# facebookresearch/hyperreel

Hardware: NVIDIA H100
Metric: Mrays/s at 65k-ray x 32-sample batch (higher is better)
Workload: dtype f32 (sample net bf16x3 split on wgmma, fp32 accumulate)

## Files before the change

hyperreel_b200/csrc/hr_mlp.cuh:

```cuda
#pragma once
#include <cuda_runtime.h>
#include "hyperreel_b200.h"

namespace hr {

struct MlpSimtPack {
  const float* Wt[HR_MAX_LAYERS];
  const float* bias[HR_MAX_LAYERS];
  int Kp[HR_MAX_LAYERS];
  int Np[HR_MAX_LAYERS];
  int in_pad;
  int n_layers;
  int skip;
};

#define HR_TC_MAX_PASSES 40
struct TcPass {
  int layer;
  int n;
  int first_chunk;
  int n_chunks;
  int bias_off;
  int is_final;
  int out_col0;
  int wait_a;
};
struct MlpTcPack {
  const void* wpack;
  const float* bias;
  long long wpack_bytes;
  int n_passes;
  int bias_count;
  int in_chunks;
  TcPass passes[HR_TC_MAX_PASSES];
};

size_t mlp_simt_smem_bytes(const MlpSimtPack& pk, int W);
cudaError_t launch_mlp_simt(const hr_config& cfg, const MlpSimtPack& pk, const float* rays, float* heads,
                            long long n, int num_sms, cudaStream_t stream);

cudaError_t launch_mlp_tc2(const hr_config& cfg, const MlpTcPack& pk, const float* rays, float* heads, long long n,
                           int num_sms, cudaStream_t stream, float* rays_copy = nullptr);

struct TrainSave {
  float* enc;
  float* act;
  long long act_stride;
  int ld_enc;
};
cudaError_t launch_mlp_tc2_train(const hr_config& cfg, const MlpTcPack& pk, const float* rays, float* heads, long long n,
                                 int num_sms, cudaStream_t stream, const TrainSave& sv);

struct TrainNetLayout {
  size_t enc, act, act_stride, dlast, dy[2], part, dbpart, total;
  int ld_enc;
};
TrainNetLayout train_net_layout(const hr_config& c, long long n, int num_sms);
cudaError_t train_net_backward(const hr_config& c, const MlpSimtPack& simt, long long n, float* const* weight,
                               float* const* bias, uint8_t* ws, int num_sms, cudaStream_t st);
}

struct hr_handle;
struct hr_params;
namespace hr {
int pack_mlp_tc2(hr_handle* h, const hr_config& c, MlpTcPack& pk, size_t& alloc_bytes, int& alloc_bias,
                 const float* const* w_dev, const float* const* b_dev, cudaStream_t st);
void free_mlp_tc2(hr_handle* h);
}
```

hyperreel_b200/csrc/hr_mlp_tc2.cu:

```cuda
#include <cuda.h>
#include <cuda_bf16.h>

#include <cstdio>
#include <cstdlib>
#include <cstring>

#include "hr_encode.cuh"
#include "hr_handle.h"
#include "hr_tc_prims.cuh"

namespace hr {

namespace tc2 {
using namespace tc;

constexpr int NSTAGE = 4;
constexpr int STAGE_BYTES = 8192;
constexpr int KSTEP_BYTES = 4096;
constexpr int CONSUMERS = 2;
constexpr int NTHREADS = (CONSUMERS + 1) * 128;
constexpr int PRODUCER_REGS = 40;
constexpr int CONSUMER_REGS = 232;
static_assert(128 * PRODUCER_REGS + CONSUMERS * 128 * CONSUMER_REGS <= 65536, "register file");

constexpr int A_BYTES = 16 * KSTEP_BYTES;
constexpr int OFF_AHI = 0;
constexpr int OFF_ALO = OFF_AHI + A_BYTES;
constexpr int X_BYTES = 4 * KSTEP_BYTES;
constexpr int OFF_X = OFF_ALO + A_BYTES;
constexpr int OFF_B = OFF_X + 2 * X_BYTES;
constexpr int OFF_BAR = OFF_B + CONSUMERS * NSTAGE * STAGE_BYTES;
constexpr int SMEM_BYTES = OFF_BAR + 128;
static_assert(SMEM_BYTES <= 232448, "shared memory budget");

constexpr int BAR_FULL = 0;
constexpr int BAR_EMPTY = BAR_FULL + CONSUMERS * NSTAGE;
static_assert((BAR_EMPTY + CONSUMERS * NSTAGE) * 8 <= 128, "barrier block");

constexpr int NB_RET = 3;
constexpr int NB_WR = 5;
constexpr int NB_XW = 7;
constexpr int NB_XR = 9;

}

template <int W, bool SAVE>
__global__ void __launch_bounds__(tc2::NTHREADS, 1)
mlp_tc2_kernel(const __grid_constant__ hr_config cfg, const __grid_constant__ MlpTcPack pk, const float* __restrict__ rays,
               float* __restrict__ heads, long long n_rays, float* __restrict__ rays_copy, const TrainSave sv) {
  using namespace tc2;
  constexpr int WH = W / 2;
  constexpr int NACC = WH / 2;
  constexpr int NK = W / 16;
  constexpr int NKH = NK / 2;
  constexpr int IMG_BYTES = WH * 64;
  constexpr int KPS = STAGE_BYTES / IMG_BYTES;
  static_assert(KPS * IMG_BYTES == STAGE_BYTES && NKH % KPS == 0 && NK * KSTEP_BYTES <= A_BYTES, "pass width");
  extern __shared__ __align__(128) uint8_t smem[];
  const uint32_t sbase = smem_u32(smem);
  const int tid = threadIdx.x, warp = tid >> 5, lane = tid & 31;
  auto bar = [&](int slot) -> uint32_t { return sbase + OFF_BAR + slot * 8; };

  {
    const char* w = reinterpret_cast<const char*>(pk.wpack);
    const long long lines = pk.wpack_bytes >> 7;
    for (long long i = (long long)blockIdx.x * NTHREADS + tid; i < lines; i += (long long)gridDim.x * NTHREADS)
      asm volatile("prefetch.global.L2 [%0];" ::"l"(w + i * 128));
  }
  for (int i = tid; i < (2 * X_BYTES) / 16; i += NTHREADS)
    reinterpret_cast<uint4*>(smem + OFF_X)[i] = make_uint4(0u, 0u, 0u, 0u);
  if (tid == 0) {
    for (int s = 0; s < CONSUMERS * NSTAGE; ++s) { mbar_init(bar(BAR_FULL + s), 1); mbar_init(bar(BAR_EMPTY + s), 1); }
    asm volatile("fence.mbarrier_init.release.cluster;" ::: "memory");
  }
  __syncthreads();

  const long long n_tiles = (n_rays + BM - 1) / BM;
  const int n_passes = pk.n_passes;
  const long long n_iters = ((long long)blockIdx.x < n_tiles) ? (n_tiles - 1 - blockIdx.x) / gridDim.x + 1 : 0;

  if (warp >= CONSUMERS * 4) {
    setmaxnreg_dec<PRODUCER_REGS>();
    const int g = warp - CONSUMERS * 4;
    if (g < CONSUMERS && lane == 0) {
      const long long half_bytes = pk.wpack_bytes / CONSUMERS;
      const int n_stages = (int)(half_bytes / STAGE_BYTES);
      const uint32_t full0 = bar(BAR_FULL + g * NSTAGE), empty0 = bar(BAR_EMPTY + g * NSTAGE);
      const uint32_t ring = sbase + OFF_B + (uint32_t)(g * NSTAGE * STAGE_BYTES);
      uint32_t stage = 0, phase = 0;
      for (long long iter = 0; iter < n_iters; ++iter) {
        const uint8_t* src = reinterpret_cast<const uint8_t*>(pk.wpack) + g * half_bytes;
        for (int i = 0; i < n_stages; ++i) {
          mbar_wait(empty0 + stage * 8, phase ^ 1);
          mbar_expect_tx(full0 + stage * 8, STAGE_BYTES);
          bulk_g2s(ring + stage * STAGE_BYTES, src, STAGE_BYTES, full0 + stage * 8);
          src += STAGE_BYTES;
          if (++stage == NSTAGE) { stage = 0; phase ^= 1; }
        }
      }
    }
    return;
  }

  setmaxnreg_inc<CONSUMER_REGS>();
  const int wg = warp >> 2;
  const int wt = tid & 127;
  const int rowq = (warp & 3) * 16 + (lane >> 2);
  const int q2 = (lane & 3) * 2;
  const int col0 = wg * WH;
  const int in_chunks = pk.in_chunks;
  const int L = cfg.mlp_layers;
  const uint32_t x_lo_off = (uint32_t)(2 * in_chunks * KSTEP_BYTES);
  const uint32_t full0 = bar(BAR_FULL + wg * NSTAGE), empty0 = bar(BAR_EMPTY + wg * NSTAGE);
  const uint32_t ring = sbase + OFF_B + (uint32_t)(wg * NSTAGE * STAGE_BYTES);
  const bool vec_ok = ((reinterpret_cast<uintptr_t>(rays) | reinterpret_cast<uintptr_t>(rays_copy)) & 15) == 0;
  int x_last = 0;
  for (int p = 0; p < n_passes; ++p)
    if (pk.passes[p].first_chunk == 0) x_last = p;
  uint32_t stage = 0, phase = 0;
  int pend = -1;

  float acc[2][NACC];

  auto stage_begin = [&]() {
    mbar_wait(full0 + stage * 8, phase);
    wgmma_fence();
    acc_fence(acc[0]);
    acc_fence(acc[1]);
  };
  auto stage_end = [&]() {
    wgmma_commit();
    acc_fence(acc[0]);
    acc_fence(acc[1]);
    wgmma_wait<1>();
    if (pend >= 0 && wt == 0) mbar_arrive(empty0 + pend * 8);
    pend = (int)stage;
    if (++stage == NSTAGE) { stage = 0; phase ^= 1; }
  };
  auto b_img = [&](int sub) -> uint32_t { return ring + stage * STAGE_BYTES + (uint32_t)sub * IMG_BYTES; };
  auto kstep = [&](uint32_t a, uint32_t a_lo, uint32_t b, uint32_t scale) {
    const uint64_t bh = gmma_desc(b, WH * 16, 128), bl = gmma_desc(b + WH * 32, WH * 16, 128);
    const uint64_t ah0 = gmma_desc(a, 2048, 128), ah1 = gmma_desc(a + 1024, 2048, 128);
    const uint64_t al0 = gmma_desc(a + a_lo, 2048, 128), al1 = gmma_desc(a + a_lo + 1024, 2048, 128);
    wgmma_ss(acc[0], ah0, bh, scale);
    wgmma_ss(acc[1], ah1, bh, scale);
    wgmma_ss(acc[0], al0, bh, 1u);
    wgmma_ss(acc[1], al1, bh, 1u);
    wgmma_ss(acc[0], ah0, bl, 1u);
    wgmma_ss(acc[1], ah1, bl, 1u);
  };
  auto run_pass = [&](const TcPass& P, bool fresh, bool x_ret, bool ret) {
    int ki = 0;
    if (P.first_chunk == 0) {
      for (; ki < 2 * in_chunks; ki += KPS) {
        stage_begin();
#pragma unroll
        for (int sub = 0; sub < KPS; ++sub)
          kstep(sbase + OFF_X + (uint32_t)(ki + sub) * KSTEP_BYTES, x_lo_off, b_img(sub), (ki + sub) != 0 ? 1u : 0u);
        stage_end();
      }
    }
    if (P.first_chunk + P.n_chunks > in_chunks) {
      const uint32_t scale0 = ki != 0 ? 1u : 0u;
#pragma unroll
      for (int kk = 0; kk < NK; ++kk) {
        if (kk % KPS == 0) {
          if (fresh && kk == (wg == 0 ? NKH : 0)) {
            if (wg == 0) pair_arrive(NB_WR + 0);
            pair_wait(NB_WR + (wg ^ 1));
          }
          stage_begin();
        }
        kstep(sbase + OFF_AHI + (uint32_t)kk * KSTEP_BYTES, OFF_ALO - OFF_AHI, b_img(kk % KPS), kk != 0 ? 1u : scale0);
        if (kk % KPS == KPS - 1) {
          stage_end();
          if (x_ret && kk == KPS - 1) pair_arrive(NB_XR + wg);
          if (ret && wg == 1 && kk == NKH + KPS - 1) pair_arrive(NB_RET + 1);
        }
      }
    }
  };
  auto drain = [&]() {
    wgmma_wait<0>();
    acc_fence(acc[0]);
    acc_fence(acc[1]);
    if (pend >= 0 && wt == 0) mbar_arrive(empty0 + pend * 8);
    pend = -1;
  };
  const int st_row = (warp & 3) * 16 + 8 * ((lane >> 3) & 1) + (lane & 7);
  const uint32_t st_off = ks_slot(st_row, lane >> 4);
  auto store_hidden = [&](const float* bias, int layer, long long tile) {
#pragma unroll
    for (int kk = 0; kk < NKH; ++kk) {
      float2 b[2];
#pragma unroll
      for (int jj = 0; jj < 2; ++jj) b[jj] = __ldg(reinterpret_cast<const float2*>(bias + col0 + 8 * (2 * kk + jj) + q2));
#pragma unroll
      for (int m = 0; m < 2; ++m) {
        uint32_t hi[4], lo[4];
#pragma unroll
        for (int jj = 0; jj < 2; ++jj) {
          const int j = 2 * kk + jj, k = col0 + 8 * j + q2;
#pragma unroll
          for (int h = 0; h < 2; ++h) {
            float t0 = acc[m][4 * j + 2 * h] + b[jj].x, t1 = acc[m][4 * j + 2 * h + 1] + b[jj].y;
            t0 = fmaxf(t0, t0 * cfg.leaky_slope);
            t1 = fmaxf(t1, t1 * cfg.leaky_slope);
            split2(t0, t1, hi[2 * jj + h], lo[2 * jj + h]);
            if constexpr (SAVE) {
              const long long ray = tile * BM + 64 * m + rowq + 8 * h;
              if (ray < n_rays) *reinterpret_cast<float2*>(sv.act + layer * sv.act_stride + ray * W + k) = make_float2(t0, t1);
            }
          }
        }
        const uint32_t a = sbase + st_off + (uint32_t)m * 1024u + (uint32_t)(wg * NKH + kk) * KSTEP_BYTES;
        stmatrix_x4(a + OFF_AHI, hi);
        stmatrix_x4(a + OFF_ALO, lo);
      }
    }
  };
  auto encode = [&](long long tile, bool after_x) {
    if (after_x) pair_wait(NB_XR + (wg ^ 1));
    const int r = wg * 64 + (wt & 63), part = wt >> 6;
    const long long ray = tile * BM + r;
    auto put = [&](int k, float val) {
      if constexpr (SAVE) {
        if (ray < n_rays) sv.enc[ray * sv.ld_enc + k] = val;
      }
      const __nv_bfloat16 hi = __float2bfloat16_rn(val);
      const __nv_bfloat16 lo = __float2bfloat16_rn(val - __bfloat162float(hi));
      const uint32_t off = (uint32_t)(k >> 4) * KSTEP_BYTES + ks_slot(r, (k >> 3) & 1) + (uint32_t)(k & 7) * 2u;
      *reinterpret_cast<__nv_bfloat16*>(smem + OFF_X + off) = hi;
      *reinterpret_cast<__nv_bfloat16*>(smem + OFF_X + x_lo_off + off) = lo;
    };
    if (ray < n_rays) {
      float rbuf[16];
      const float* src = rays + ray * cfg.c_in;
      if (cfg.c_in == 8 && vec_ok) {
        const float4 a = *reinterpret_cast<const float4*>(src), b = *reinterpret_cast<const float4*>(src + 4);
        rbuf[0] = a.x; rbuf[1] = a.y; rbuf[2] = a.z; rbuf[3] = a.w; rbuf[4] = b.x; rbuf[5] = b.y; rbuf[6] = b.z; rbuf[7] = b.w;
        if (rays_copy != nullptr && part == 0) {
          float4* dst = reinterpret_cast<float4*>(rays_copy + ray * 8);
          dst[0] = a; dst[1] = b;
        }
      } else {
        for (int i = 0; i < cfg.c_in; ++i) rbuf[i] = src[i];
        if (rays_copy != nullptr && part == 0)
          for (int i = 0; i < cfg.c_in; ++i) rays_copy[ray * cfg.c_in + i] = rbuf[i];
      }
      encode_ray_features(cfg, rbuf, part, 2, put);
      if constexpr (SAVE) {
        if (part == 0)
          for (int k = cfg.mlp_in; k < sv.ld_enc; ++k) sv.enc[ray * sv.ld_enc + k] = 0.0f;
      }
    } else if (part == 0) {
      for (int k = 0; k < cfg.mlp_in; ++k) put(k, 0.0f);
    }
    fence_async_smem();
    wg_sync(1 + wg);
    pair_arrive(NB_XW + wg);
  };

  for (long long iter = 0; iter < n_iters; ++iter) {
    const long long tile = iter * gridDim.x + blockIdx.x;
    const bool more = iter + 1 < n_iters;
    if (iter == 0) encode(tile, false);
    pair_wait(NB_XW + (wg ^ 1));
    for (int p = 0; p < n_passes; ++p) {
      const TcPass& P = pk.passes[p];
      const bool reads_a = P.first_chunk + P.n_chunks > in_chunks;
      const bool hidden = p < L - 1;
      const bool ret = reads_a && (hidden || (p == n_passes - 1 && more));
      const bool x_ret = p == x_last && more;
      run_pass(P, reads_a && P.wait_a != 0, x_ret, ret);
      drain();
      if (x_ret && !reads_a) pair_arrive(NB_XR + wg);
      if (ret && wg == 0) pair_arrive(NB_RET + 0);
      if (hidden) {
        wg_sync(1 + wg);
        if (p > 0 || iter > 0) pair_wait(NB_RET + (wg ^ 1));
        store_hidden(pk.bias + P.bias_off, p, tile);
        fence_async_smem();
        wg_sync(1 + wg);
        if (wg == 1) pair_arrive(NB_WR + 1);
      } else {
        const float* bias = pk.bias + P.bias_off;
        if constexpr (SAVE) {
#pragma unroll
          for (int m = 0; m < 2; ++m)
#pragma unroll
            for (int h = 0; h < 2; ++h) {
              const long long ray = tile * BM + 64 * m + rowq + 8 * h;
              if (ray >= n_rays) continue;
              float* row = heads + ray * cfg.mlp_out;
#pragma unroll
              for (int j = 0; j < WH / 8; ++j) {
                const int c = col0 + 8 * j + q2;
                if (P.out_col0 + c < cfg.mlp_out) {
                  const float2 b = __ldg(reinterpret_cast<const float2*>(bias + c));
                  const int c0 = P.out_col0 + c, c1 = c0 + 1, S = cfg.n_samples;
                  row[(c0 % S) * cfg.head_stride + c0 / S] = acc[m][4 * j + 2 * h] + b.x;
                  row[(c1 % S) * cfg.head_stride + c1 / S] = acc[m][4 * j + 2 * h + 1] + b.y;
                }
              }
            }
        } else {
          const bool odd = (lane & 1) != 0;
#pragma unroll
          for (int jp = 0; jp < WH / 16; ++jp) {
            const int j = 2 * jp, c = col0 + 8 * j + q2;
            const float2 b0 = __ldg(reinterpret_cast<const float2*>(bias + c));
            const float2 b1 = __ldg(reinterpret_cast<const float2*>(bias + c + 8));
#pragma unroll
            for (int m = 0; m < 2; ++m)
#pragma unroll
              for (int h = 0; h < 2; ++h) {
                const float2 v0 = make_float2(acc[m][4 * j + 2 * h] + b0.x, acc[m][4 * j + 2 * h + 1] + b0.y);
                const float2 v1 = make_float2(acc[m][4 * j + 4 + 2 * h] + b1.x, acc[m][4 * j + 4 + 2 * h + 1] + b1.y);
                const float2 send = odd ? v0 : v1;
                const float2 recv = make_float2(__shfl_xor_sync(0xffffffffu, send.x, 1), __shfl_xor_sync(0xffffffffu, send.y, 1));
                const int c4 = odd ? c + 6 : c;
                const long long ray = tile * BM + 64 * m + rowq + 8 * h;
                if (ray < n_rays && P.out_col0 + c4 < cfg.mlp_out)
                  *reinterpret_cast<float4*>(heads + ray * cfg.mlp_out + P.out_col0 + c4) =
                      odd ? make_float4(recv.x, recv.y, v1.x, v1.y) : make_float4(v0.x, v0.y, recv.x, recv.y);
              }
          }
        }
      }
      if (x_ret) encode(tile + gridDim.x, true);
    }
  }
}

int pack_mlp_tc2(hr_handle* h, const hr_config& c, MlpTcPack& pk, size_t& alloc_bytes, int& alloc_bias,
                 const float* const* w_dev, const float* const* b_dev, cudaStream_t st) {
  const int W = c.mlp_width;
  if (W != 128 && W != 256) return hr_fail("tensor-core sample net: hidden width must be 128 or 256 (got %d)", W);
  if (c.mlp_in > 64) return hr_fail("tensor-core sample net: encoded input wider than 64 features (%d)", c.mlp_in);
  const int in_chunks = (c.mlp_in + 31) / 32;
  const int L = c.mlp_layers;
  MlpTcPack np_{};
  np_.in_chunks = in_chunks;
  int np = 0, bias_off = 0;
  size_t bytes = 0;
  for (int l = 0; l < L; ++l) {
    const bool last = (l == L - 1);
    const int out = last ? c.mlp_out : W;
    const int n_parts = (out + W - 1) / W;
    for (int part = 0; part < n_parts; ++part) {
      if (np >= HR_TC_MAX_PASSES) return hr_fail("tensor-core sample net: too many passes (%d output columns)", c.mlp_out);
      TcPass& P = np_.passes[np++];
      const bool reads_input = (l == 0 || l == c.mlp_skip);
      P.layer = l;
      P.n = W;
      P.first_chunk = reads_input ? 0 : in_chunks;
      P.n_chunks = (l == 0) ? in_chunks : (W / 32 + (reads_input ? in_chunks : 0));
      P.bias_off = bias_off;
      P.is_final = last ? 1 : 0;
      P.out_col0 = part * W;
      P.wait_a = (part == 0) ? 1 : 0;
      bias_off += P.n;
      bytes += (size_t)P.n_chunks * 2 * P.n * 64;
    }
  }
  np_.n_passes = np;
  np_.bias_count = bias_off;
  np_.wpack_bytes = (long long)bytes;
  if (alloc_bytes != bytes || alloc_bias != bias_off || !pk.wpack) {
    if (pk.wpack) cudaFree(const_cast<void*>(pk.wpack));
    if (pk.bias) cudaFree(const_cast<float*>(pk.bias));
    pk.wpack = nullptr; pk.bias = nullptr;
    alloc_bytes = 0; alloc_bias = 0;
    void* wp = nullptr; float* bp = nullptr;
    cudaError_t e = cudaMalloc(&wp, bytes);
    if (e != cudaSuccess) return hr_fail("cudaMalloc(tc weights %zu): %s", bytes, cudaGetErrorString(e));
    e = cudaMalloc((void**)&bp, (size_t)bias_off * sizeof(float));
    if (e != cudaSuccess) { cudaFree(wp); return hr_fail("cudaMalloc(tc bias): %s", cudaGetErrorString(e)); }
    np_.wpack = wp; np_.bias = bp;
    alloc_bytes = bytes; alloc_bias = bias_off;
    e = (W == 256) ? cudaFuncSetAttribute(mlp_tc2_kernel<256, false>, cudaFuncAttributeMaxDynamicSharedMemorySize, tc2::SMEM_BYTES)
                   : cudaFuncSetAttribute(mlp_tc2_kernel<128, false>, cudaFuncAttributeMaxDynamicSharedMemorySize, tc2::SMEM_BYTES);
    if (e != cudaSuccess) return hr_fail("cudaFuncSetAttribute(mlp_tc2_kernel): %s", cudaGetErrorString(e));
  } else {
    np_.wpack = pk.wpack; np_.bias = pk.bias;
  }
  pk = np_;
  uint8_t* wp = (uint8_t*)const_cast<void*>(pk.wpack);
  float* bp = const_cast<float*>(pk.bias);
  const int WH = W / 2;
  for (int half = 0; half < 2; ++half) {
    size_t off = (size_t)half * (bytes / 2);
    for (int p = 0; p < np; ++p) {
      const TcPass& P = pk.passes[p];
      const int l = P.layer;
      const bool last = (l == L - 1), skip = (l == c.mlp_skip), first = (l == 0);
      const int in_src = first ? c.mlp_in : (skip ? c.mlp_in + W : W);
      launch_pack_tc_pass(w_dev[l], b_dev[l], wp + off, bp + P.bias_off + half * WH, WH, P.first_chunk, P.n_chunks, in_src,
                          c.mlp_in, skip ? 1 : 0, in_chunks, last ? c.mlp_out : W, last ? c.n_samples : 0, c.head_stride,
                          P.out_col0 + half * WH, st);
      off += (size_t)P.n_chunks * 2 * WH * 64;
    }
  }
  cudaError_t e = cudaGetLastError();
  if (e != cudaSuccess) return hr_fail("tc pack launch failed: %s", cudaGetErrorString(e));
  return 0;
}

void free_mlp_tc2(hr_handle* h) {
  if (h->tc.wpack) cudaFree(const_cast<void*>(h->tc.wpack));
  if (h->tc.bias) cudaFree(const_cast<float*>(h->tc.bias));
  h->tc.wpack = nullptr; h->tc.bias = nullptr;
  h->tc_alloc_bytes = 0; h->tc_alloc_bias = 0;
  if (h->tc_pre.wpack) cudaFree(const_cast<void*>(h->tc_pre.wpack));
  if (h->tc_pre.bias) cudaFree(const_cast<float*>(h->tc_pre.bias));
  h->tc_pre.wpack = nullptr; h->tc_pre.bias = nullptr;
  h->tc_pre_alloc_bytes = 0; h->tc_pre_alloc_bias = 0;
}

cudaError_t launch_mlp_tc2(const hr_config& cfg, const MlpTcPack& pk, const float* rays, float* heads, long long n, int num_sms,
                           cudaStream_t stream, float* rays_copy) {
  if ((cfg.mlp_out % 4) != 0 || ((uintptr_t)heads % 16) != 0) return cudaErrorInvalidValue;
  long long tiles = (n + tc::BM - 1) / tc::BM;
  int grid = (int)(tiles < num_sms ? tiles : num_sms);
  if (grid < 1) grid = 1;
  if (cfg.mlp_width == 256)
    mlp_tc2_kernel<256, false><<<grid, tc2::NTHREADS, tc2::SMEM_BYTES, stream>>>(cfg, pk, rays, heads, n, rays_copy, TrainSave{});
  else if (cfg.mlp_width == 128)
    mlp_tc2_kernel<128, false><<<grid, tc2::NTHREADS, tc2::SMEM_BYTES, stream>>>(cfg, pk, rays, heads, n, rays_copy, TrainSave{});
  else
    return cudaErrorInvalidValue;
  return cudaGetLastError();
}

cudaError_t launch_mlp_tc2_train(const hr_config& cfg, const MlpTcPack& pk, const float* rays, float* heads, long long n,
                                 int num_sms, cudaStream_t stream, const TrainSave& sv) {
  if ((cfg.mlp_out % 4) != 0) return cudaErrorInvalidValue;
  long long tiles = (n + tc::BM - 1) / tc::BM;
  int grid = (int)(tiles < num_sms ? tiles : num_sms);
  if (grid < 1) grid = 1;
  auto kern = cfg.mlp_width == 256 ? mlp_tc2_kernel<256, true> : mlp_tc2_kernel<128, true>;
  if (cfg.mlp_width != 256 && cfg.mlp_width != 128) return cudaErrorInvalidValue;
  cudaError_t e = cudaFuncSetAttribute(kern, cudaFuncAttributeMaxDynamicSharedMemorySize, tc2::SMEM_BYTES);
  if (e != cudaSuccess) return e;
  kern<<<grid, tc2::NTHREADS, tc2::SMEM_BYTES, stream>>>(cfg, pk, rays, heads, n, nullptr, sv);
  return cudaGetLastError();
}

}
```

hyperreel_b200/csrc/hr_tc_pack.cu:

```cuda
#include <cuda_bf16.h>

#include "hr_tc_prims.cuh"

namespace hr {

__global__ void pack_tc_pass(const float* __restrict__ W, const float* __restrict__ b, uint8_t* __restrict__ dst,
                             float* __restrict__ bias_dst, int n, int first_chunk, int n_chunks, int in_src, int mlp_in,
                             int is_skip, int in_chunks, int out_rows, int perm_S, int perm_stride, int out_col0) {
  const long long total = (long long)n_chunks * 2 * n * 16;
  for (long long i = blockIdx.x * (long long)blockDim.x + threadIdx.x; i < total + n; i += (long long)gridDim.x * blockDim.x) {
    if (i >= total) {
      int nn = (int)(i - total);
      int ncol = out_col0 + nn;
      float v = 0.0f;
      if (ncol < out_rows) {
        int ns = perm_S > 0 ? (ncol % perm_S) * perm_stride + (ncol / perm_S) : ncol;
        v = b[ns];
      }
      bias_dst[nn] = v;
      continue;
    }
    int kk = (int)(i % 16);
    int nn = (int)((i / 16) % n);
    int img = (int)(i / (16LL * n));
    int c = first_chunk + img / 2, ks = img % 2;
    int kc = ks * 16 + kk;
    int ksrc = -1;
    if (c < in_chunks) {
      const int kin = c * 32 + kc;
      if (kin < mlp_in) ksrc = kin;
    } else {
      int hcol = (c - in_chunks) * 32 + kc;
      ksrc = is_skip ? mlp_in + hcol : hcol;
    }
    int ncol = out_col0 + nn;
    float w = 0.0f;
    if (ncol < out_rows && ksrc >= 0 && ksrc < in_src) {
      int ns = perm_S > 0 ? (ncol % perm_S) * perm_stride + (ncol / perm_S) : ncol;
      w = W[(long long)ns * in_src + ksrc];
    }
    __nv_bfloat16 hi = __float2bfloat16_rn(w);
    __nv_bfloat16 lo = __float2bfloat16_rn(w - __bfloat162float(hi));
    size_t img_off = (size_t)img * n * 64;
    size_t slot = (size_t)(((kk >> 3) * (n >> 3) + (nn >> 3)) * 128 + (nn & 7) * 16 + (kk & 7) * 2);
    *reinterpret_cast<__nv_bfloat16*>(dst + img_off + slot) = hi;
    *reinterpret_cast<__nv_bfloat16*>(dst + img_off + (size_t)n * 32 + slot) = lo;
  }
}

void launch_pack_tc_pass(const float* W, const float* b, uint8_t* dst, float* bias_dst, int n, int first_chunk, int n_chunks,
                         int in_src, int mlp_in, int is_skip, int in_chunks, int out_rows, int perm_S, int perm_stride,
                         int out_col0, cudaStream_t st) {
  long long total = (long long)n_chunks * 2 * n * 16 + n;
  int grid = (int)((total + 255) / 256);
  if (grid > 4096) grid = 4096;
  pack_tc_pass<<<grid, 256, 0, st>>>(W, b, dst, bias_dst, n, first_chunk, n_chunks, in_src, mlp_in, is_skip, in_chunks, out_rows,
                                     perm_S, perm_stride, out_col0);
}

}
```

hyperreel_b200/csrc/hr_tc_prims.cuh:

```cuda
#pragma once
#include <cuda.h>
#include <cuda_bf16.h>
#include <stdint.h>

namespace hr {
namespace tc {

constexpr int BM = 128;

__device__ __forceinline__ uint32_t smem_u32(const void* p) { return (uint32_t)__cvta_generic_to_shared(p); }

__device__ __forceinline__ void mbar_init(uint32_t bar, uint32_t count) {
  asm volatile("mbarrier.init.shared::cta.b64 [%0], %1;" ::"r"(bar), "r"(count) : "memory");
}
__device__ __forceinline__ void mbar_arrive(uint32_t bar) {
  asm volatile("{\n\t.reg .b64 st;\n\tmbarrier.arrive.shared::cta.b64 st, [%0];\n\t}" ::"r"(bar) : "memory");
}
__device__ __forceinline__ void mbar_expect_tx(uint32_t bar, uint32_t bytes) {
  asm volatile("{\n\t.reg .b64 st;\n\tmbarrier.arrive.expect_tx.shared::cta.b64 st, [%0], %1;\n\t}" ::"r"(bar), "r"(bytes)
               : "memory");
}
__device__ __forceinline__ void mbar_wait(uint32_t bar, uint32_t parity) {
  asm volatile(
      "{\n\t"
      ".reg .pred p;\n\t"
      "WAIT_LOOP:\n\t"
      "mbarrier.try_wait.parity.shared::cta.b64 p, [%0], %1;\n\t"
      "@p bra DONE;\n\t"
      "bra WAIT_LOOP;\n\t"
      "DONE:\n\t"
      "}" ::"r"(bar), "r"(parity)
      : "memory");
}
__device__ __forceinline__ void bulk_g2s(uint32_t dst, const void* src, uint32_t bytes, uint32_t bar) {
  asm volatile("cp.async.bulk.shared::cluster.global.mbarrier::complete_tx::bytes [%0], [%1], %2, [%3];" ::"r"(dst), "l"(src),
               "r"(bytes), "r"(bar)
               : "memory");
}
__device__ __forceinline__ void fence_async_smem() { asm volatile("fence.proxy.async.shared::cta;" ::: "memory"); }
__device__ __forceinline__ void wg_sync(int id) { asm volatile("bar.sync %0, 128;" ::"r"(id) : "memory"); }
__device__ __forceinline__ void pair_arrive(int id) { asm volatile("bar.arrive %0, 256;" ::"r"(id) : "memory"); }
__device__ __forceinline__ void pair_wait(int id) { asm volatile("bar.sync %0, 256;" ::"r"(id) : "memory"); }

__device__ __forceinline__ uint64_t gmma_desc(uint32_t saddr, uint32_t lbo_bytes, uint32_t sbo_bytes) {
  uint64_t d = 0;
  d |= (uint64_t)((saddr & 0x3FFFF) >> 4);
  d |= (uint64_t)((lbo_bytes >> 4) & 0x3FFF) << 16;
  d |= (uint64_t)((sbo_bytes >> 4) & 0x3FFF) << 32;
  return d;
}

__device__ __forceinline__ void wgmma_fence() { asm volatile("wgmma.fence.sync.aligned;" ::: "memory"); }
__device__ __forceinline__ void wgmma_commit() { asm volatile("wgmma.commit_group.sync.aligned;" ::: "memory"); }
template <int N>
__device__ __forceinline__ void wgmma_wait() {
  asm volatile("wgmma.wait_group.sync.aligned %0;" ::"n"(N) : "memory");
}
template <int N>
__device__ __forceinline__ void acc_fence(float (&d)[N]) {
#pragma unroll
  for (int i = 0; i < N; ++i) asm volatile("" : "+f"(d[i])::"memory");
}
template <int R>
__device__ __forceinline__ void setmaxnreg_dec() { asm volatile("setmaxnreg.dec.sync.aligned.u32 %0;" ::"n"(R)); }
template <int R>
__device__ __forceinline__ void setmaxnreg_inc() { asm volatile("setmaxnreg.inc.sync.aligned.u32 %0;" ::"n"(R)); }

__device__ __forceinline__ void wgmma_ss(float (&d)[32], uint64_t adesc, uint64_t bdesc, uint32_t accumulate) {
  asm volatile(
      "{\n\t"
      ".reg .pred p;\n\t"
      "setp.ne.b32 p, %34, 0;\n\t"
      "wgmma.mma_async.sync.aligned.m64n64k16.f32.bf16.bf16 "
      "{"
      "%0, %1, %2, %3, %4, %5, %6, %7, %8, %9, %10, %11, %12, %13, %14, %15, %16, %17, %18, %19, %20, %21, %22, "
      "%23, %24, %25, %26, %27, %28, %29, %30, %31"
      "}, %32, %33, p, 1, 1, 0, 0;\n\t"
      "}"
      : "+f"(d[0]), "+f"(d[1]), "+f"(d[2]), "+f"(d[3]), "+f"(d[4]), "+f"(d[5]), "+f"(d[6]), "+f"(d[7]),
        "+f"(d[8]), "+f"(d[9]), "+f"(d[10]), "+f"(d[11]), "+f"(d[12]), "+f"(d[13]), "+f"(d[14]), "+f"(d[15]),
        "+f"(d[16]), "+f"(d[17]), "+f"(d[18]), "+f"(d[19]), "+f"(d[20]), "+f"(d[21]), "+f"(d[22]), "+f"(d[23]),
        "+f"(d[24]), "+f"(d[25]), "+f"(d[26]), "+f"(d[27]), "+f"(d[28]), "+f"(d[29]), "+f"(d[30]), "+f"(d[31])
      : "l"(adesc), "l"(bdesc), "r"(accumulate));
}

__device__ __forceinline__ void wgmma_ss(float (&d)[64], uint64_t adesc, uint64_t bdesc, uint32_t accumulate) {
  asm volatile(
      "{\n\t"
      ".reg .pred p;\n\t"
      "setp.ne.b32 p, %66, 0;\n\t"
      "wgmma.mma_async.sync.aligned.m64n128k16.f32.bf16.bf16 "
      "{"
      "%0, %1, %2, %3, %4, %5, %6, %7, %8, %9, %10, %11, %12, %13, %14, %15, %16, %17, %18, %19, %20, %21, %22, "
      "%23, %24, %25, %26, %27, %28, %29, %30, %31, %32, %33, %34, %35, %36, %37, %38, %39, %40, %41, %42, %43, "
      "%44, %45, %46, %47, %48, %49, %50, %51, %52, %53, %54, %55, %56, %57, %58, %59, %60, %61, %62, %63"
      "}, %64, %65, p, 1, 1, 0, 0;\n\t"
      "}"
      : "+f"(d[0]), "+f"(d[1]), "+f"(d[2]), "+f"(d[3]), "+f"(d[4]), "+f"(d[5]), "+f"(d[6]), "+f"(d[7]),
        "+f"(d[8]), "+f"(d[9]), "+f"(d[10]), "+f"(d[11]), "+f"(d[12]), "+f"(d[13]), "+f"(d[14]), "+f"(d[15]),
        "+f"(d[16]), "+f"(d[17]), "+f"(d[18]), "+f"(d[19]), "+f"(d[20]), "+f"(d[21]), "+f"(d[22]), "+f"(d[23]),
        "+f"(d[24]), "+f"(d[25]), "+f"(d[26]), "+f"(d[27]), "+f"(d[28]), "+f"(d[29]), "+f"(d[30]), "+f"(d[31]),
        "+f"(d[32]), "+f"(d[33]), "+f"(d[34]), "+f"(d[35]), "+f"(d[36]), "+f"(d[37]), "+f"(d[38]), "+f"(d[39]),
        "+f"(d[40]), "+f"(d[41]), "+f"(d[42]), "+f"(d[43]), "+f"(d[44]), "+f"(d[45]), "+f"(d[46]), "+f"(d[47]),
        "+f"(d[48]), "+f"(d[49]), "+f"(d[50]), "+f"(d[51]), "+f"(d[52]), "+f"(d[53]), "+f"(d[54]), "+f"(d[55]),
        "+f"(d[56]), "+f"(d[57]), "+f"(d[58]), "+f"(d[59]), "+f"(d[60]), "+f"(d[61]), "+f"(d[62]), "+f"(d[63])
      : "l"(adesc), "l"(bdesc), "r"(accumulate));
}

__device__ __forceinline__ void stmatrix_x4(uint32_t addr, const uint32_t (&r)[4]) {
  asm volatile("stmatrix.sync.aligned.m8n8.x4.shared.b16 [%0], {%1, %2, %3, %4};" ::"r"(addr), "r"(r[0]), "r"(r[1]), "r"(r[2]),
               "r"(r[3])
               : "memory");
}

__device__ __forceinline__ uint32_t ks_slot(int row, int kg) { return (uint32_t)((kg * 16 + (row >> 3)) * 128 + (row & 7) * 16); }

__device__ __forceinline__ void split2(float x0, float x1, uint32_t& hi, uint32_t& lo) {
  __nv_bfloat162 hh = __floats2bfloat162_rn(x0, x1);
  __nv_bfloat162 ll = __floats2bfloat162_rn(x0 - __low2float(hh), x1 - __high2float(hh));
  hi = *reinterpret_cast<uint32_t*>(&hh);
  lo = *reinterpret_cast<uint32_t*>(&ll);
}

}

void launch_pack_tc_pass(const float* W, const float* b, uint8_t* dst, float* bias_dst, int n, int first_chunk, int n_chunks,
                         int in_src, int mlp_in, int is_skip, int in_chunks, int out_rows, int perm_S, int perm_stride,
                         int out_col0, cudaStream_t st);
}
```

Before: 155.0.

## Trim final-layer wgmma width and input k-steps to actual sizes

Passes now carry a per-pass output half-width (nh) and a k-step count, so the last partial output pass issues narrower wgmma shapes (n32/n48/n96/n112) instead of full-width ones. The input k range is padded to a KPS multiple of 16-wide steps rather than 32-wide chunks. The producer streams variable-sized stages that match each pass. Together these aim to cut wasted tensor-core work and weight bytes on padded columns and input features. The cost is extra template instantiations, per-pass dispatch, and a bias buffer padded and zeroed to cover out-of-pass reads.

```diff
diff --git a/hyperreel_b200/csrc/hr_mlp.cuh b/hyperreel_b200/csrc/hr_mlp.cuh
--- a/hyperreel_b200/csrc/hr_mlp.cuh
+++ b/hyperreel_b200/csrc/hr_mlp.cuh
@@ -17,9 +17,9 @@
 #define HR_TC_MAX_PASSES 40
 struct TcPass {
   int layer;
-  int n;
-  int first_chunk;
-  int n_chunks;
+  int nh;
+  int reads_x;
+  int n_ksteps;
   int bias_off;
   int is_final;
   int out_col0;
@@ -31,7 +31,7 @@
   long long wpack_bytes;
   int n_passes;
   int bias_count;
-  int in_chunks;
+  int in_ksteps;
   TcPass passes[HR_TC_MAX_PASSES];
 };
 
diff --git a/hyperreel_b200/csrc/hr_mlp_tc2.cu b/hyperreel_b200/csrc/hr_mlp_tc2.cu
--- a/hyperreel_b200/csrc/hr_mlp_tc2.cu
+++ b/hyperreel_b200/csrc/hr_mlp_tc2.cu
@@ -4,6 +4,7 @@
 #include <cstdio>
 #include <cstdlib>
 #include <cstring>
+#include <type_traits>
 
 #include "hr_encode.cuh"
 #include "hr_handle.h"
@@ -84,18 +85,20 @@
     const int g = warp - CONSUMERS * 4;
     if (g < CONSUMERS && lane == 0) {
       const long long half_bytes = pk.wpack_bytes / CONSUMERS;
-      const int n_stages = (int)(half_bytes / STAGE_BYTES);
       const uint32_t full0 = bar(BAR_FULL + g * NSTAGE), empty0 = bar(BAR_EMPTY + g * NSTAGE);
       const uint32_t ring = sbase + OFF_B + (uint32_t)(g * NSTAGE * STAGE_BYTES);
       uint32_t stage = 0, phase = 0;
       for (long long iter = 0; iter < n_iters; ++iter) {
         const uint8_t* src = reinterpret_cast<const uint8_t*>(pk.wpack) + g * half_bytes;
-        for (int i = 0; i < n_stages; ++i) {
-          mbar_wait(empty0 + stage * 8, phase ^ 1);
-          mbar_expect_tx(full0 + stage * 8, STAGE_BYTES);
-          bulk_g2s(ring + stage * STAGE_BYTES, src, STAGE_BYTES, full0 + stage * 8);
-          src += STAGE_BYTES;
-          if (++stage == NSTAGE) { stage = 0; phase ^= 1; }
+        for (int p = 0; p < n_passes; ++p) {
+          const uint32_t bytes = (uint32_t)(KPS * pk.passes[p].nh * 64);
+          for (int i = pk.passes[p].n_ksteps / KPS; i > 0; --i) {
+            mbar_wait(empty0 + stage * 8, phase ^ 1);
+            mbar_expect_tx(full0 + stage * 8, bytes);
+            bulk_g2s(ring + stage * STAGE_BYTES, src, bytes, full0 + stage * 8);
+            src += bytes;
+            if (++stage == NSTAGE) { stage = 0; phase ^= 1; }
+          }
         }
       }
     }
@@ -108,15 +111,15 @@
   const int rowq = (warp & 3) * 16 + (lane >> 2);
   const int q2 = (lane & 3) * 2;
   const int col0 = wg * WH;
-  const int in_chunks = pk.in_chunks;
+  const int in_ksteps = pk.in_ksteps;
   const int L = cfg.mlp_layers;
-  const uint32_t x_lo_off = (uint32_t)(2 * in_chunks * KSTEP_BYTES);
+  const uint32_t x_lo_off = (uint32_t)(in_ksteps * KSTEP_BYTES);
   const uint32_t full0 = bar(BAR_FULL + wg * NSTAGE), empty0 = bar(BAR_EMPTY + wg * NSTAGE);
   const uint32_t ring = sbase + OFF_B + (uint32_t)(wg * NSTAGE * STAGE_BYTES);
   const bool vec_ok = ((reinterpret_cast<uintptr_t>(rays) | reinterpret_cast<uintptr_t>(rays_copy)) & 15) == 0;
   int x_last = 0;
   for (int p = 0; p < n_passes; ++p)
-    if (pk.passes[p].first_chunk == 0) x_last = p;
+    if (pk.passes[p].reads_x) x_last = p;
   uint32_t stage = 0, phase = 0;
   int pend = -1;
 
@@ -137,32 +140,34 @@
     pend = (int)stage;
     if (++stage == NSTAGE) { stage = 0; phase ^= 1; }
   };
-  auto b_img = [&](int sub) -> uint32_t { return ring + stage * STAGE_BYTES + (uint32_t)sub * IMG_BYTES; };
-  auto kstep = [&](uint32_t a, uint32_t a_lo, uint32_t b, uint32_t scale) {
-    const uint64_t bh = gmma_desc(b, WH * 16, 128), bl = gmma_desc(b + WH * 32, WH * 16, 128);
+  auto kstep = [&](uint32_t a, uint32_t a_lo, uint32_t b, uint32_t scale, auto nb) {
+    constexpr int NB = decltype(nb)::value;
+    const uint64_t bh = gmma_desc(b, NB * 16, 128), bl = gmma_desc(b + NB * 32, NB * 16, 128);
     const uint64_t ah0 = gmma_desc(a, 2048, 128), ah1 = gmma_desc(a + 1024, 2048, 128);
     const uint64_t al0 = gmma_desc(a + a_lo, 2048, 128), al1 = gmma_desc(a + a_lo + 1024, 2048, 128);
-    wgmma_ss(acc[0], ah0, bh, scale);
-    wgmma_ss(acc[1], ah1, bh, scale);
-    wgmma_ss(acc[0], al0, bh, 1u);
-    wgmma_ss(acc[1], al1, bh, 1u);
-    wgmma_ss(acc[0], ah0, bl, 1u);
-    wgmma_ss(acc[1], ah1, bl, 1u);
-  };
-  auto run_pass = [&](const TcPass& P, bool fresh, bool x_ret, bool ret) {
+    wgmma_ss_cols<NB>(acc[0], ah0, bh, scale);
+    wgmma_ss_cols<NB>(acc[1], ah1, bh, scale);
+    wgmma_ss_cols<NB>(acc[0], al0, bh, 1u);
+    wgmma_ss_cols<NB>(acc[1], al1, bh, 1u);
+    wgmma_ss_cols<NB>(acc[0], ah0, bl, 1u);
+    wgmma_ss_cols<NB>(acc[1], ah1, bl, 1u);
+  };
+  auto run_pass = [&](const TcPass& P, bool fresh, bool x_ret, bool ret, auto nb) {
+    constexpr int NB = decltype(nb)::value;
+    auto b_img = [&](int sub) -> uint32_t { return ring + stage * STAGE_BYTES + (uint32_t)(sub * NB * 64); };
     int ki = 0;
-    if (P.first_chunk == 0) {
-      for (; ki < 2 * in_chunks; ki += KPS) {
+    if (P.reads_x) {
+      for (; ki < in_ksteps; ki += KPS) {
         stage_begin();
 #pragma unroll
         for (int sub = 0; sub < KPS; ++sub)
-          kstep(sbase + OFF_X + (uint32_t)(ki + sub) * KSTEP_BYTES, x_lo_off, b_img(sub), (ki + sub) != 0 ? 1u : 0u);
+          kstep(sbase + OFF_X + (uint32_t)(ki + sub) * KSTEP_BYTES, x_lo_off, b_img(sub), (ki + sub) != 0 ? 1u : 0u, nb);
         stage_end();
       }
     }
-    if (P.first_chunk + P.n_chunks > in_chunks) {
+    if (P.layer != 0) {
       const uint32_t scale0 = ki != 0 ? 1u : 0u;
-#pragma unroll
+#pragma unroll (NB == WH || W == 128 ? NK : 1)
       for (int kk = 0; kk < NK; ++kk) {
         if (kk % KPS == 0) {
           if (fresh && kk == (wg == 0 ? NKH : 0)) {
@@ -171,7 +176,7 @@
           }
           stage_begin();
         }
-        kstep(sbase + OFF_AHI + (uint32_t)kk * KSTEP_BYTES, OFF_ALO - OFF_AHI, b_img(kk % KPS), kk != 0 ? 1u : scale0);
+        kstep(sbase + OFF_AHI + (uint32_t)kk * KSTEP_BYTES, OFF_ALO - OFF_AHI, b_img(kk % KPS), kk != 0 ? 1u : scale0, nb);
         if (kk % KPS == KPS - 1) {
           stage_end();
           if (x_ret && kk == KPS - 1) pair_arrive(NB_XR + wg);
@@ -268,11 +273,14 @@
     pair_wait(NB_XW + (wg ^ 1));
     for (int p = 0; p < n_passes; ++p) {
       const TcPass& P = pk.passes[p];
-      const bool reads_a = P.first_chunk + P.n_chunks > in_chunks;
+      const bool reads_a = P.layer != 0;
       const bool hidden = p < L - 1;
       const bool ret = reads_a && (hidden || (p == n_passes - 1 && more));
       const bool x_ret = p == x_last && more;
-      run_pass(P, reads_a && P.wait_a != 0, x_ret, ret);
+      const bool fresh = reads_a && P.wait_a != 0;
+      if (P.nh == WH) run_pass(P, fresh, x_ret, ret, std::integral_constant<int, WH>{});
+      else if (P.nh == WH - 16) run_pass(P, fresh, x_ret, ret, std::integral_constant<int, WH - 16>{});
+      else run_pass(P, fresh, x_ret, ret, std::integral_constant<int, WH - 32>{});
       drain();
       if (x_ret && !reads_a) pair_arrive(NB_XR + wg);
       if (ret && wg == 0) pair_arrive(NB_RET + 0);
@@ -285,6 +293,7 @@
         if (wg == 1) pair_arrive(NB_WR + 1);
       } else {
         const float* bias = pk.bias + P.bias_off;
+        const int nh = P.nh, c0g = wg * nh;
         if constexpr (SAVE) {
 #pragma unroll
           for (int m = 0; m < 2; ++m)
@@ -295,8 +304,8 @@
               float* row = heads + ray * cfg.mlp_out;
 #pragma unroll
               for (int j = 0; j < WH / 8; ++j) {
-                const int c = col0 + 8 * j + q2;
-                if (P.out_col0 + c < cfg.mlp_out) {
+                const int c = c0g + 8 * j + q2;
+                if (8 * j < nh && P.out_col0 + c < cfg.mlp_out) {
                   const float2 b = __ldg(reinterpret_cast<const float2*>(bias + c));
                   const int c0 = P.out_col0 + c, c1 = c0 + 1, S = cfg.n_samples;
                   row[(c0 % S) * cfg.head_stride + c0 / S] = acc[m][4 * j + 2 * h] + b.x;
@@ -308,7 +317,8 @@
           const bool odd = (lane & 1) != 0;
 #pragma unroll
           for (int jp = 0; jp < WH / 16; ++jp) {
-            const int j = 2 * jp, c = col0 + 8 * j + q2;
+            const bool in_pass = 16 * jp < nh;
+            const int j = 2 * jp, c = c0g + 8 * j + q2;
             const float2 b0 = __ldg(reinterpret_cast<const float2*>(bias + c));
             const float2 b1 = __ldg(reinterpret_cast<const float2*>(bias + c + 8));
 #pragma unroll
@@ -321,7 +331,7 @@
                 const float2 recv = make_float2(__shfl_xor_sync(0xffffffffu, send.x, 1), __shfl_xor_sync(0xffffffffu, send.y, 1));
                 const int c4 = odd ? c + 6 : c;
                 const long long ray = tile * BM + 64 * m + rowq + 8 * h;
-                if (ray < n_rays && P.out_col0 + c4 < cfg.mlp_out)
+                if (in_pass && ray < n_rays && P.out_col0 + c4 < cfg.mlp_out)
                   *reinterpret_cast<float4*>(heads + ray * cfg.mlp_out + P.out_col0 + c4) =
                       odd ? make_float4(recv.x, recv.y, v1.x, v1.y) : make_float4(v0.x, v0.y, recv.x, recv.y);
               }
@@ -338,10 +348,12 @@
   const int W = c.mlp_width;
   if (W != 128 && W != 256) return hr_fail("tensor-core sample net: hidden width must be 128 or 256 (got %d)", W);
   if (c.mlp_in > 64) return hr_fail("tensor-core sample net: encoded input wider than 64 features (%d)", c.mlp_in);
-  const int in_chunks = (c.mlp_in + 31) / 32;
+  const int WH = W / 2;
+  const int kps = tc2::STAGE_BYTES / (WH * 64);
+  const int in_ksteps = ((c.mlp_in + 15) / 16 + kps - 1) / kps * kps;
   const int L = c.mlp_layers;
   MlpTcPack np_{};
-  np_.in_chunks = in_chunks;
+  np_.in_ksteps = in_ksteps;
   int np = 0, bias_off = 0;
   size_t bytes = 0;
   for (int l = 0; l < L; ++l) {
@@ -352,16 +364,19 @@
       if (np >= HR_TC_MAX_PASSES) return hr_fail("tensor-core sample net: too many passes (%d output columns)", c.mlp_out);
       TcPass& P = np_.passes[np++];
       const bool reads_input = (l == 0 || l == c.mlp_skip);
+      const int rem = out - part * W;
+      int nh = rem >= W ? WH : ((rem + 1) / 2 + 15) / 16 * 16;
+      if (nh < WH - 32) nh = WH - 32;
       P.layer = l;
-      P.n = W;
-      P.first_chunk = reads_input ? 0 : in_chunks;
-      P.n_chunks = (l == 0) ? in_chunks : (W / 32 + (reads_input ? in_chunks : 0));
+      P.nh = nh;
+      P.reads_x = reads_input ? 1 : 0;
+      P.n_ksteps = (reads_input ? in_ksteps : 0) + (l != 0 ? W / 16 : 0);
       P.bias_off = bias_off;
       P.is_final = last ? 1 : 0;
       P.out_col0 = part * W;
       P.wait_a = (part == 0) ? 1 : 0;
-      bias_off += P.n;
-      bytes += (size_t)P.n_chunks * 2 * P.n * 64;
+      bias_off += 2 * nh;
+      bytes += (size_t)P.n_ksteps * 2 * nh * 64;
     }
   }
   np_.n_passes = np;
@@ -375,8 +390,11 @@
     void* wp = nullptr; float* bp = nullptr;
     cudaError_t e = cudaMalloc(&wp, bytes);
     if (e != cudaSuccess) return hr_fail("cudaMalloc(tc weights %zu): %s", bytes, cudaGetErrorString(e));
-    e = cudaMalloc((void**)&bp, (size_t)bias_off * sizeof(float));
+    const size_t bias_alloc = ((size_t)bias_off + 32) * sizeof(float);
+    e = cudaMalloc((void**)&bp, bias_alloc);
     if (e != cudaSuccess) { cudaFree(wp); return hr_fail("cudaMalloc(tc bias): %s", cudaGetErrorString(e)); }
+    e = cudaMemsetAsync(bp, 0, bias_alloc, st);
+    if (e != cudaSuccess) { cudaFree(wp); cudaFree(bp); return hr_fail("cudaMemsetAsync(tc bias): %s", cudaGetErrorString(e)); }
     np_.wpack = wp; np_.bias = bp;
     alloc_bytes = bytes; alloc_bias = bias_off;
     e = (W == 256) ? cudaFuncSetAttribute(mlp_tc2_kernel<256, false>, cudaFuncAttributeMaxDynamicSharedMemorySize, tc2::SMEM_BYTES)
@@ -388,7 +406,6 @@
   pk = np_;
   uint8_t* wp = (uint8_t*)const_cast<void*>(pk.wpack);
   float* bp = const_cast<float*>(pk.bias);
-  const int WH = W / 2;
   for (int half = 0; half < 2; ++half) {
     size_t off = (size_t)half * (bytes / 2);
     for (int p = 0; p < np; ++p) {
@@ -396,10 +413,10 @@
       const int l = P.layer;
       const bool last = (l == L - 1), skip = (l == c.mlp_skip), first = (l == 0);
       const int in_src = first ? c.mlp_in : (skip ? c.mlp_in + W : W);
-      launch_pack_tc_pass(w_dev[l], b_dev[l], wp + off, bp + P.bias_off + half * WH, WH, P.first_chunk, P.n_chunks, in_src,
-                          c.mlp_in, skip ? 1 : 0, in_chunks, last ? c.mlp_out : W, last ? c.n_samples : 0, c.head_stride,
-                          P.out_col0 + half * WH, st);
-      off += (size_t)P.n_chunks * 2 * WH * 64;
+      launch_pack_tc_pass(w_dev[l], b_dev[l], wp + off, bp + P.bias_off + half * P.nh, P.nh, P.reads_x, P.n_ksteps, in_src,
+                          c.mlp_in, skip ? 1 : 0, in_ksteps, last ? c.mlp_out : W, last ? c.n_samples : 0, c.head_stride,
+                          P.out_col0 + half * P.nh, st);
+      off += (size_t)P.n_ksteps * P.nh * 64;
     }
   }
   cudaError_t e = cudaGetLastError();
diff --git a/hyperreel_b200/csrc/hr_tc_pack.cu b/hyperreel_b200/csrc/hr_tc_pack.cu
--- a/hyperreel_b200/csrc/hr_tc_pack.cu
+++ b/hyperreel_b200/csrc/hr_tc_pack.cu
@@ -5,9 +5,9 @@
 namespace hr {
 
 __global__ void pack_tc_pass(const float* __restrict__ W, const float* __restrict__ b, uint8_t* __restrict__ dst,
-                             float* __restrict__ bias_dst, int n, int first_chunk, int n_chunks, int in_src, int mlp_in,
-                             int is_skip, int in_chunks, int out_rows, int perm_S, int perm_stride, int out_col0) {
-  const long long total = (long long)n_chunks * 2 * n * 16;
+                             float* __restrict__ bias_dst, int n, int reads_x, int n_ksteps, int in_src, int mlp_in,
+                             int is_skip, int in_ksteps, int out_rows, int perm_S, int perm_stride, int out_col0) {
+  const long long total = (long long)n_ksteps * n * 16;
   for (long long i = blockIdx.x * (long long)blockDim.x + threadIdx.x; i < total + n; i += (long long)gridDim.x * blockDim.x) {
     if (i >= total) {
       int nn = (int)(i - total);
@@ -23,14 +23,12 @@
     int kk = (int)(i % 16);
     int nn = (int)((i / 16) % n);
     int img = (int)(i / (16LL * n));
-    int c = first_chunk + img / 2, ks = img % 2;
-    int kc = ks * 16 + kk;
     int ksrc = -1;
-    if (c < in_chunks) {
-      const int kin = c * 32 + kc;
+    if (reads_x && img < in_ksteps) {
+      const int kin = img * 16 + kk;
       if (kin < mlp_in) ksrc = kin;
     } else {
-      int hcol = (c - in_chunks) * 32 + kc;
+      int hcol = (img - (reads_x ? in_ksteps : 0)) * 16 + kk;
       ksrc = is_skip ? mlp_in + hcol : hcol;
     }
     int ncol = out_col0 + nn;
@@ -48,13 +46,13 @@
   }
 }
 
-void launch_pack_tc_pass(const float* W, const float* b, uint8_t* dst, float* bias_dst, int n, int first_chunk, int n_chunks,
-                         int in_src, int mlp_in, int is_skip, int in_chunks, int out_rows, int perm_S, int perm_stride,
+void launch_pack_tc_pass(const float* W, const float* b, uint8_t* dst, float* bias_dst, int n, int reads_x, int n_ksteps,
+                         int in_src, int mlp_in, int is_skip, int in_ksteps, int out_rows, int perm_S, int perm_stride,
                          int out_col0, cudaStream_t st) {
-  long long total = (long long)n_chunks * 2 * n * 16 + n;
+  long long total = (long long)n_ksteps * n * 16 + n;
   int grid = (int)((total + 255) / 256);
   if (grid > 4096) grid = 4096;
-  pack_tc_pass<<<grid, 256, 0, st>>>(W, b, dst, bias_dst, n, first_chunk, n_chunks, in_src, mlp_in, is_skip, in_chunks, out_rows,
+  pack_tc_pass<<<grid, 256, 0, st>>>(W, b, dst, bias_dst, n, reads_x, n_ksteps, in_src, mlp_in, is_skip, in_ksteps, out_rows,
                                      perm_S, perm_stride, out_col0);
 }
 
diff --git a/hyperreel_b200/csrc/hr_tc_prims.cuh b/hyperreel_b200/csrc/hr_tc_prims.cuh
--- a/hyperreel_b200/csrc/hr_tc_prims.cuh
+++ b/hyperreel_b200/csrc/hr_tc_prims.cuh
@@ -107,6 +107,100 @@
       : "l"(adesc), "l"(bdesc), "r"(accumulate));
 }
 
+template <int R>
+__device__ __forceinline__ void wgmma_ss_n32(float (&d)[R], uint64_t adesc, uint64_t bdesc, uint32_t accumulate) {
+  static_assert(R >= 16, "accumulator");
+  asm volatile(
+      "{\n\t"
+      ".reg .pred p;\n\t"
+      "setp.ne.b32 p, %18, 0;\n\t"
+      "wgmma.mma_async.sync.aligned.m64n32k16.f32.bf16.bf16 "
+      "{"
+      "%0, %1, %2, %3, %4, %5, %6, %7, %8, %9, %10, %11, %12, %13, %14, %15"
+      "}, %16, %17, p, 1, 1, 0, 0;\n\t"
+      "}"
+      : "+f"(d[0]), "+f"(d[1]), "+f"(d[2]), "+f"(d[3]), "+f"(d[4]), "+f"(d[5]), "+f"(d[6]), "+f"(d[7]),
+        "+f"(d[8]), "+f"(d[9]), "+f"(d[10]), "+f"(d[11]), "+f"(d[12]), "+f"(d[13]), "+f"(d[14]), "+f"(d[15])
+      : "l"(adesc), "l"(bdesc), "r"(accumulate));
+}
+
+template <int R>
+__device__ __forceinline__ void wgmma_ss_n48(float (&d)[R], uint64_t adesc, uint64_t bdesc, uint32_t accumulate) {
+  static_assert(R >= 24, "accumulator");
+  asm volatile(
+      "{\n\t"
+      ".reg .pred p;\n\t"
+      "setp.ne.b32 p, %26, 0;\n\t"
+      "wgmma.mma_async.sync.aligned.m64n48k16.f32.bf16.bf16 "
+      "{"
+      "%0, %1, %2, %3, %4, %5, %6, %7, %8, %9, %10, %11, %12, %13, %14, %15, %16, %17, %18, %19, %20, %21, "
+      "%22, %23"
+      "}, %24, %25, p, 1, 1, 0, 0;\n\t"
+      "}"
+      : "+f"(d[0]), "+f"(d[1]), "+f"(d[2]), "+f"(d[3]), "+f"(d[4]), "+f"(d[5]), "+f"(d[6]), "+f"(d[7]),
+        "+f"(d[8]), "+f"(d[9]), "+f"(d[10]), "+f"(d[11]), "+f"(d[12]), "+f"(d[13]), "+f"(d[14]), "+f"(d[15]),
+        "+f"(d[16]), "+f"(d[17]), "+f"(d[18]), "+f"(d[19]), "+f"(d[20]), "+f"(d[21]), "+f"(d[22]), "+f"(d[23])
+      : "l"(adesc), "l"(bdesc), "r"(accumulate));
+}
+
+template <int R>
+__device__ __forceinline__ void wgmma_ss_n96(float (&d)[R], uint64_t adesc, uint64_t bdesc, uint32_t accumulate) {
+  static_assert(R >= 48, "accumulator");
+  asm volatile(
+      "{\n\t"
+      ".reg .pred p;\n\t"
+      "setp.ne.b32 p, %50, 0;\n\t"
+      "wgmma.mma_async.sync.aligned.m64n96k16.f32.bf16.bf16 "
+      "{"
+      "%0, %1, %2, %3, %4, %5, %6, %7, %8, %9, %10, %11, %12, %13, %14, %15, %16, %17, %18, %19, %20, %21, "
+      "%22, %23, %24, %25, %26, %27, %28, %29, %30, %31, %32, %33, %34, %35, %36, %37, %38, %39, %40, %41, "
+      "%42, %43, %44, %45, %46, %47"
+      "}, %48, %49, p, 1, 1, 0, 0;\n\t"
+      "}"
+      : "+f"(d[0]), "+f"(d[1]), "+f"(d[2]), "+f"(d[3]), "+f"(d[4]), "+f"(d[5]), "+f"(d[6]), "+f"(d[7]),
+        "+f"(d[8]), "+f"(d[9]), "+f"(d[10]), "+f"(d[11]), "+f"(d[12]), "+f"(d[13]), "+f"(d[14]), "+f"(d[15]),
+        "+f"(d[16]), "+f"(d[17]), "+f"(d[18]), "+f"(d[19]), "+f"(d[20]), "+f"(d[21]), "+f"(d[22]), "+f"(d[23]),
+        "+f"(d[24]), "+f"(d[25]), "+f"(d[26]), "+f"(d[27]), "+f"(d[28]), "+f"(d[29]), "+f"(d[30]), "+f"(d[31]),
+        "+f"(d[32]), "+f"(d[33]), "+f"(d[34]), "+f"(d[35]), "+f"(d[36]), "+f"(d[37]), "+f"(d[38]), "+f"(d[39]),
+        "+f"(d[40]), "+f"(d[41]), "+f"(d[42]), "+f"(d[43]), "+f"(d[44]), "+f"(d[45]), "+f"(d[46]), "+f"(d[47])
+      : "l"(adesc), "l"(bdesc), "r"(accumulate));
+}
+
+template <int R>
+__device__ __forceinline__ void wgmma_ss_n112(float (&d)[R], uint64_t adesc, uint64_t bdesc, uint32_t accumulate) {
+  static_assert(R >= 56, "accumulator");
+  asm volatile(
+      "{\n\t"
+      ".reg .pred p;\n\t"
+      "setp.ne.b32 p, %58, 0;\n\t"
+      "wgmma.mma_async.sync.aligned.m64n112k16.f32.bf16.bf16 "
+      "{"
+      "%0, %1, %2, %3, %4, %5, %6, %7, %8, %9, %10, %11, %12, %13, %14, %15, %16, %17, %18, %19, %20, %21, "
+      "%22, %23, %24, %25, %26, %27, %28, %29, %30, %31, %32, %33, %34, %35, %36, %37, %38, %39, %40, %41, "
+      "%42, %43, %44, %45, %46, %47, %48, %49, %50, %51, %52, %53, %54, %55"
+      "}, %56, %57, p, 1, 1, 0, 0;\n\t"
+      "}"
+      : "+f"(d[0]), "+f"(d[1]), "+f"(d[2]), "+f"(d[3]), "+f"(d[4]), "+f"(d[5]), "+f"(d[6]), "+f"(d[7]),
+        "+f"(d[8]), "+f"(d[9]), "+f"(d[10]), "+f"(d[11]), "+f"(d[12]), "+f"(d[13]), "+f"(d[14]), "+f"(d[15]),
+        "+f"(d[16]), "+f"(d[17]), "+f"(d[18]), "+f"(d[19]), "+f"(d[20]), "+f"(d[21]), "+f"(d[22]), "+f"(d[23]),
+        "+f"(d[24]), "+f"(d[25]), "+f"(d[26]), "+f"(d[27]), "+f"(d[28]), "+f"(d[29]), "+f"(d[30]), "+f"(d[31]),
+        "+f"(d[32]), "+f"(d[33]), "+f"(d[34]), "+f"(d[35]), "+f"(d[36]), "+f"(d[37]), "+f"(d[38]), "+f"(d[39]),
+        "+f"(d[40]), "+f"(d[41]), "+f"(d[42]), "+f"(d[43]), "+f"(d[44]), "+f"(d[45]), "+f"(d[46]), "+f"(d[47]),
+        "+f"(d[48]), "+f"(d[49]), "+f"(d[50]), "+f"(d[51]), "+f"(d[52]), "+f"(d[53]), "+f"(d[54]), "+f"(d[55])
+      : "l"(adesc), "l"(bdesc), "r"(accumulate));
+}
+
+template <int N, int R>
+__device__ __forceinline__ void wgmma_ss_cols(float (&d)[R], uint64_t adesc, uint64_t bdesc, uint32_t accumulate) {
+  static_assert(N % 16 == 0 && N <= 2 * R, "wgmma width");
+  if constexpr (N == 2 * R) wgmma_ss(d, adesc, bdesc, accumulate);
+  else if constexpr (N == 32) wgmma_ss_n32(d, adesc, bdesc, accumulate);
+  else if constexpr (N == 48) wgmma_ss_n48(d, adesc, bdesc, accumulate);
+  else if constexpr (N == 96) wgmma_ss_n96(d, adesc, bdesc, accumulate);
+  else if constexpr (N == 112) wgmma_ss_n112(d, adesc, bdesc, accumulate);
+  else static_assert(N == 2 * R, "no wgmma instantiated for this width");
+}
+
 __device__ __forceinline__ void stmatrix_x4(uint32_t addr, const uint32_t (&r)[4]) {
   asm volatile("stmatrix.sync.aligned.m8n8.x4.shared.b16 [%0], {%1, %2, %3, %4};" ::"r"(addr), "r"(r[0]), "r"(r[1]), "r"(r[2]),
                "r"(r[3])
@@ -124,7 +218,7 @@
 
 }
 
-void launch_pack_tc_pass(const float* W, const float* b, uint8_t* dst, float* bias_dst, int n, int first_chunk, int n_chunks,
-                         int in_src, int mlp_in, int is_skip, int in_chunks, int out_rows, int perm_S, int perm_stride,
+void launch_pack_tc_pass(const float* W, const float* b, uint8_t* dst, float* bias_dst, int n, int reads_x, int n_ksteps,
+                         int in_src, int mlp_in, int is_skip, int in_ksteps, int out_rows, int perm_S, int perm_stride,
                          int out_col0, cudaStream_t st);
 }
```

After: 154.6, median of 6. About the same (-0.2%).
